# A-Kokolis/Hermes

Hardware: AMD Instinct MI355X
Metric: replicated KVS ops/s (reads+writes committed) (higher is better)
Workload: dtype u8

## Files before the change

hermes_amd/csrc/hkv_batch_dev.h:

```cpp
#pragma once
#include <hip/hip_runtime.h>

#include <type_traits>

#include "hkv_exec.h"
#include "hkv_internal.h"
#include "hkv_table_dev.h"

namespace hkv {

constexpr uint32_t kNone = 0xFFFFFFFFu;
enum : uint8_t { kStDone = 0, kStCommit = 1, kStPend = 2, kStDefer = 3 };
enum { kCtrFbM = 1, kCtrFbL = 2, kCtrDefer = 3 };

struct BatchArgs {
    uint8_t *elems;
    const int32_t *counts;
    const int32_t *offsets;
    const uint8_t *index;
    uint8_t *log;
    uint8_t *rw;
    int32_t *ns_idx;
    unsigned long long *fw;
    unsigned long long *fx, *fy;
    unsigned long long *ft;
    uint32_t fw_mask;
    uint32_t *ent;
    uint8_t *st;
    uint32_t *pf;
    uint8_t *shadow;
    unsigned long long *mem;
    uint32_t *fbl;
    uint32_t *ctr;
    unsigned int *error_flags;
    Geometry g;
    int64_t n;
    int64_t rw_stride;
    int32_t stride;
    int32_t esz;
    int32_t type;
    uint32_t rtag0;
    uint8_t ltag;
    int32_t rounds;
    int32_t inv_direct;
    int32_t ack_direct;
    uint8_t g_membership;
    uint8_t w_ack_init;
    int32_t *node_suspected;
    int32_t n_batches;
    const uint8_t *host_src;
    uint8_t *host_dst;
    uint8_t *dev_region;
    uint64_t region_bytes;
    uint32_t *done_flag;
    uint32_t done_value;
    unsigned long long *prof;
    const SmallBatch *hdr;
    uint8_t *state_out;
    const uint8_t *opc;
    const uint8_t *patch;
    uint16_t *fk;
    uint64_t *hx;
    uint8_t *rws;
    const uint8_t *rwo;
    int32_t n_rows, skip_row;
    int64_t row_stride;
    int32_t dbg;
    int32_t check_unique;
    uint8_t *ack_out;
    uint32_t ack_out_size;
    uint8_t *line;
};

enum class Engine : uint8_t {
    kSmall,
    kLocalDirect,
    kRows,
    kUniqueLds64,
    kUniqueLdsBig,
    kUniqueInPlace,
    kValsOnePass,
    kRoundsAckDirect,
    kRoundsInvDirect,
    kRoundsSlab,
    kRoundsInPlace,
};
enum class Patches : uint8_t {
    kNone,
    kApplyFirst,
    kByEngine,
    kInResolve,
};
constexpr uint32_t kPirMaxValue = 320;
constexpr uint32_t kWaveWordsMaxValue = 8 * 62;
static_assert(kPirMaxValue <= kWaveWordsMaxValue, "wave_value_copies_n ignores VCopy::fill: handle it there first");
struct BatchPlan {
    int refuse;
    Engine engine;
    Patches patches;
    int sv;
    int rmax, ch;
    int slab_threads;
    int64_t lookup_head;
    bool big;
    bool mixed;
    bool inv_direct, ack_direct;
    bool ack_out;
    bool state_out, opc;
    bool fk;
    bool rw_mirrors;
    bool node_suspected;
    bool il;
    bool inline_instance;
};

int launch_small(const BatchArgs &a, const BatchPlan &p, hipStream_t s);
int launch_local(const BatchArgs &a, const BatchPlan &p, hipStream_t s);

template <class F>
inline void with_sv(int sv, F &&f)
{
    if (sv == 31) f(std::integral_constant<int, 31>{});
    else if (sv == 287) f(std::integral_constant<int, 287>{});
    else f(std::integral_constant<int, 0>{});
}
template <class F>
inline void with_bool(bool b, F &&f)
{
    if (b) f(std::true_type{});
    else f(std::false_type{});
}

__device__ __forceinline__ Ctx make_ctx(const BatchArgs &a)
{
    Ctx c;
    c.g = a.g;
    c.g_membership = a.g_membership;
    c.w_ack_init = a.w_ack_init;
    c.rw = nullptr;
    c.rws = nullptr;
    c.rw_done = nullptr;
    c.vc = nullptr;
    return c;
}

__device__ __forceinline__ uint64_t phys_of(const BatchArgs &a, uint32_t e) { return (uint64_t)e * a.g.entry_unit; }
__device__ __forceinline__ uint8_t *entry_of(const BatchArgs &a, uint32_t e) { return a.log + phys_of(a, e); }

struct __attribute__((aligned(8))) U64x2 {
    uint64_t a, b;
};

template <int TYPE>
__device__ __forceinline__ uint8_t absorbing_state()
{
    return TYPE == kVals ? kValid : kWrite;
}

template <int TYPE>
__device__ __forceinline__ Meta after_first(const BatchArgs &a, const Meta &m0, uint32_t f, int f_is_put)
{
    Meta m1 = m0;
    m_set_state(m1, absorbing_state<TYPE>());
    if (TYPE != kLocal || a.g.skew == 0) return m1;
    uint8_t foc = f_is_put ? (uint8_t)kOpPut : a.elems[(int64_t)f * a.esz + 8];
    if (a.hx && !f_is_put) {
        const uint64_t pb = *reinterpret_cast<const uint64_t *>(a.patch + (int64_t)f * 16 + 8);
        if ((pb >> 48) & 0xFFu) foc = (uint8_t)pb;
    }
    if (foc != kOpGet) {
        m1.ver += 2;
        m_set_cid(m1, (uint8_t)a.g.machine_id);
    } else {
        m_set_state(m1, kReplay);
    }
    return m1;
}

__device__ __forceinline__ int32_t batch_of(const BatchArgs &a, int64_t i, int64_t &start)
{
    if (!a.offsets) {
        const int32_t b = (int32_t)(i / a.stride);
        start = (int64_t)b * a.stride;
        return b;
    }
    int lo = 0, hi = a.n_batches - 1;
    while (lo < hi) {
        const int mid = (lo + hi + 1) >> 1;
        if (a.offsets[mid] <= i) lo = mid; else hi = mid - 1;
    }
    start = a.offsets[lo];
    return lo;
}

constexpr int kRowsWindow = 128;
__host__ __device__ inline int32_t kary_stride(int32_t lo, int32_t hi) { return (hi - lo + 63) >> 6; }
__host__ __device__ inline int32_t kary_sample(int32_t lo, int32_t hi, int s) { return lo + (s + 1) * kary_stride(lo, hi); }
__host__ __device__ inline void kary_narrow(int32_t &lo, int32_t &hi, int32_t c)
{
    const int32_t step = kary_stride(lo, hi);
    lo += c * step;
    if (lo + step - 1 < hi) hi = lo + step - 1;
}
template <class Count>
__host__ __device__ inline int32_t kary_last_le(int32_t n, int32_t span, Count &&count)
{
    int32_t lo = 0, hi = n - 1;
    while (hi - lo > span) kary_narrow(lo, hi, count(lo, hi));
    return lo;
}

template <class Win>
__host__ __device__ inline bool rows_window_batch(Win &&win, int32_t lo, int32_t k0, int64_t i, int64_t i_max, int32_t &b)
{
    int32_t k = k0;
    for (int32_t j = k0 + 1; j < kRowsWindow; ++j) {
        const int32_t v = win(j);
        if ((int64_t)v > i_max) break;
        if ((int64_t)v <= i) k = j;
    }
    b = lo + k;
    return k + 1 < kRowsWindow;
}

__device__ __forceinline__ void batch_rw(const BatchArgs &a, int32_t b, Ctx &c)
{
    c.rw = a.rw ? a.rw + (int64_t)b * a.rw_stride : nullptr;
    c.rws = a.rws ? a.rws + (int64_t)b * (a.rw_stride / a.g.op_size) : nullptr;
    c.rwo = a.rwo ? a.rwo + (int64_t)b * (a.rw_stride / a.g.op_size) : nullptr;
}

__device__ __forceinline__ void elem_at(const BatchArgs &a, uint32_t i, uint8_t *&x, uint8_t &idx, Ctx &c)
{
    c.rw = nullptr;
    c.rws = nullptr;
    idx = 0;
    if (a.rw || !a.offsets) {
        int64_t start;
        const int32_t b = batch_of(a, i, start);
        idx = (uint8_t)(i - start);
        batch_rw(a, b, c);
    }
    x = a.elems + (int64_t)i * a.esz;
}

__device__ __forceinline__ void note_state(const BatchArgs &a, int64_t i, const uint8_t *x)
{
    if (a.state_out) a.state_out[i] = x[9];
}

__device__ __forceinline__ uint32_t fw_index(const BatchArgs &a, uint64_t phys)
{
    return (uint32_t)(((phys >> 6) * 0x9E3779B1ull) & a.fw_mask);
}
__device__ __forceinline__ unsigned long long *fw_of(const BatchArgs &a, uint32_t e) { return a.fw + fw_index(a, phys_of(a, e)); }

__device__ __forceinline__ uint32_t first_cand(unsigned long long f, uint32_t rtag)
{
    return (uint32_t)(f >> 32) == ~rtag ? (uint32_t)f : kNone;
}

__device__ __forceinline__ void offer(unsigned long long *f, uint32_t rtag, uint32_t i)
{
    const unsigned long long v = ((unsigned long long)(~rtag) << 32) | i;
    if (v < __hip_atomic_load(f, __ATOMIC_RELAXED, __HIP_MEMORY_SCOPE_AGENT)) atomicMin(f, v);
}

__device__ __forceinline__ uint8_t *shadow_of(const BatchArgs &a, uint32_t i)
{
    return a.shadow + (size_t)i * a.g.entry_size;
}

__device__ __forceinline__ void copy_entry(uint8_t *dst, const uint8_t *src, uint32_t bytes)
{
    struct __attribute__((aligned(8))) W16 {
        uint64_t a, b;
    };
    uint32_t o = 0;
    for (; o + 16 <= bytes; o += 16) *reinterpret_cast<W16 *>(dst + o) = *reinterpret_cast<const W16 *>(src + o);
    if (o < bytes) *reinterpret_cast<uint64_t *>(dst + o) = *reinterpret_cast<const uint64_t *>(src + o);
}

template <int TYPE, int SV>
__device__ __forceinline__ void apply_to_shadow(const BatchArgs &a, uint8_t *x, uint32_t i, const uint8_t *src)
{
    uint8_t *sh = shadow_of(a, i);
    Meta m;
    meta_load(src, m);
    if (SV == 31) {
        const uint4 *s4 = reinterpret_cast<const uint4 *>(src);
        uint4 *d4 = reinterpret_cast<uint4 *>(sh);
        const uint4 w0 = s4[0], w1 = s4[1], w2 = s4[2], w3 = s4[3];
        d4[0] = w0;
        d4[1] = w1;
        d4[2] = w2;
        d4[3] = w3;
    } else {
        copy_entry(sh, src, a.g.entry_size);
    }
    Ctx c = make_ctx(a);
    uint8_t *xg;
    uint8_t idx;
    elem_at(a, i, xg, idx, c);
    if (x) dispatch<SV>(TYPE, x, sh, idx, m, c);
    else dispatch<SV>(TYPE, xg, sh, idx, m, c);
    meta_store(sh, m);
}

__device__ __forceinline__ bool patch_valid(uint64_t pb) { return ((pb >> 48) & 0xFFu) != 0; }

__device__ __forceinline__ bool in_count(const BatchArgs &a, uint32_t i)
{
    if (!a.counts) return true;
    const uint32_t b = i / (uint32_t)a.stride;
    return (int32_t)(i - b * (uint32_t)a.stride) < a.counts[b];
}

__device__ __forceinline__ uint64_t line_key_meta(const uint4 &ln, Meta &m)
{
    const uint64_t ek = (uint64_t)(uint32_t)__shfl((int)ln.z, 0, 4) | ((uint64_t)(uint32_t)__shfl((int)ln.w, 0, 4) << 32);
    m.w4 = (uint32_t)__shfl((int)ln.x, 1, 4);
    m.w5 = (uint32_t)__shfl((int)ln.y, 1, 4);
    m.ver = (uint32_t)__shfl((int)ln.z, 1, 4);
    const uint32_t w7 = (uint32_t)__shfl((int)ln.w, 1, 4);
    const uint32_t b32 = (uint32_t)__shfl((int)ln.x, 2, 4) & 0xFFu;
    m.llw_cid = (uint8_t)w7;
    m.llw_ver = (w7 >> 8) | (b32 << 24);
    return ek;
}

constexpr int kLookupPair = 2;
struct NothingBeside {
    __device__ __forceinline__ void operator()() const {}
};
template <int P = kLookupPair, bool IL = false, bool F = false, class Beside = NothingBeside>
__device__ __forceinline__ void lookup_core(const BatchArgs &a, const uint64_t *key, const bool *probe, int q,
                                            int gbase, bool *ok, uint64_t *phys, uint4 *ln, unsigned long long *fwv,
                                            uint8_t **home, bool *inl, Beside &&beside = Beside{})
{
    uint4 v[P], ev[P];
#pragma unroll
    for (int k = 0; k < P; ++k) {
        if (IL) {
            const uint4 *l = line_words(a.line, bucket_of(a.g, key[k]));
            v[k] = probe[k] ? l[q] : make_uint4(0u, 0u, 0u, 0u);
            ev[k] = probe[k] ? l[4 + q] : make_uint4(0u, 0u, 0u, 0u);
        } else {
            v[k] = probe[k] ? bucket_words(a.index, bucket_of(a.g, key[k]))[q] : make_uint4(0u, 0u, 0u, 0u);
        }
    }
    beside();
    bool il[P];
#pragma unroll
    for (int k = 0; k < P; ++k) {
        const uint64_t s0 = u64_of(v[k].x, v[k].y), s1 = u64_of(v[k].z, v[k].w);
        const uint32_t tag = key_tag(key[k]);
        const bool mt0 = probe[k] && (s0 & 1u) && ((uint32_t)(s0 >> 1) & 0x7FFFFFu) == tag;
        const bool mt1 = probe[k] && (s1 & 1u) && ((uint32_t)(s1 >> 1) & 0x7FFFFFu) == tag;
        const uint32_t g0 = (uint32_t)(__ballot(mt0) >> gbase) & 0xFu;
        const uint32_t g1 = (uint32_t)(__ballot(mt1) >> gbase) & 0xFu;
        uint32_t o = 0;
#pragma unroll
        for (int l = 0; l < 4; ++l) o |= ((g0 >> l) & 1u) << (2 * l) | ((g1 >> l) & 1u) << (2 * l + 1);
        const int first = o ? __ffs(o) - 1 : 0;
        const uint64_t raw = group_slot_word(slot_off_raw(s0), slot_off_raw(s1), first), off = off_of<IL>(raw);
        ok[k] = probe[k] && o && in_log_window(a.g, off);
        phys[k] = off & a.g.log_mask;
        il[k] = off_is_inline<IL>(raw) && ok[k];
    }
#pragma unroll
    for (int k = 0; k < P; ++k) {
        if (IL) {
            ln[k] = ev[k];
            if (!il[k]) ln[k] = ok[k] ? reinterpret_cast<const uint4 *>(a.log + phys[k])[q] : make_uint4(0u, 0u, 0u, 0u);
            if (home) home[k] = il[k] ? line_entry(a.line, a.g, key[k]) : a.log + phys[k];
            if (inl) inl[k] = il[k];
        } else {
            ln[k] = ok[k] ? reinterpret_cast<const uint4 *>(a.log + phys[k])[q] : make_uint4(0u, 0u, 0u, 0u);
            if (home) home[k] = a.log + phys[k];
            if (inl) inl[k] = false;
        }
        if (F) fwv[k] = ok[k] && q == 0 ? a.fw[fw_index(a, phys[k])] : ~0ull;
    }
}

template <int P = kLookupPair, bool IL = false>
__device__ __forceinline__ void lookup_pair(const BatchArgs &a, const uint64_t *key, const bool *probe, int q,
                                            int gbase, bool *ok, uint64_t *phys, uint4 *ln, uint8_t **home = nullptr,
                                            bool *inl = nullptr)
{
    lookup_core<P, IL, false>(a, key, probe, q, gbase, ok, phys, ln, nullptr, home, inl);
}

template <int P, bool IL, class Beside>
__device__ __forceinline__ void lookup_pair_beside(const BatchArgs &a, const uint64_t *key, const bool *probe, int q,
                                                   int gbase, bool *ok, uint64_t *phys, uint4 *ln, uint8_t **home,
                                                   Beside &&beside)
{
    lookup_core<P, IL, false>(a, key, probe, q, gbase, ok, phys, ln, nullptr, home, nullptr, beside);
}

template <int P, bool IL = false>
__device__ __forceinline__ void lookup_pair_f(const BatchArgs &a, const uint64_t *key, const bool *probe, int q,
                                              int gbase, bool *ok, uint64_t *phys, uint4 *ln, unsigned long long *fwv,
                                              uint8_t **home = nullptr, bool *inl = nullptr)
{
    lookup_core<P, IL, true>(a, key, probe, q, gbase, ok, phys, ln, fwv, home, inl);
}

}
```

hermes_amd/csrc/hkv_batch_local.hip:

```cpp
#include <hip/hip_runtime.h>

#include "hkv_batch_dev.h"

namespace hkv {

#ifdef HKV_DEBUG_MODES
#define HKV_DBG_ON(a, bit) (((a).dbg & (bit)) != 0)
#else
#define HKV_DBG_ON(a, bit) false
#endif

constexpr int kPreElems = 2048;
constexpr int kPreThreads = kPreElems / 4;
constexpr int kPreHead = 1024;
constexpr int kPreHash = 2048;

constexpr uint32_t kEntInline = 0x80000000u;
template <bool IL>
__device__ __forceinline__ uint32_t ent_id(uint32_t e) { return IL ? e & ~kEntInline : e; }
template <bool IL>
__device__ __forceinline__ uint8_t *entry_home(const BatchArgs &a, uint32_t e, uint64_t key)
{
    if (IL && (e & kEntInline)) return line_entry(a.line, a.g, key);
    return entry_of(a, ent_id<IL>(e));
}

__device__ __forceinline__ uint64_t elem_key(const BatchArgs &a, int64_t i)
{
    if (a.patch && a.patch[i * 16 + 14]) return *reinterpret_cast<const uint64_t *>(a.patch + i * 16);
    return *reinterpret_cast<const uint64_t *>(a.elems + i * a.esz);
}

__device__ __forceinline__ uint4 patch_chunk(uint4 w, int q, uint64_t pa, uint64_t pb)
{
    const uint32_t fill = (uint32_t)((pb >> 32) & 0xFFu) * 0x01010101u;
    const bool vfill = fill != 0, reset = ((pb >> 40) & 0xFFu) != 0;
    if (q == 0) {
        w.x = (uint32_t)pa;
        w.y = (uint32_t)(pa >> 32);
        w.z = (uint32_t)(pb & 0xFFu) | ((uint32_t)kNew << 8) | ((uint32_t)((pb >> 8) & 0xFFu) << 16) |
              (reset ? 0u : (w.z & 0xFF000000u));
        if (reset) w.w = 0;
    } else if (q == 1) {
        const uint32_t flags = (uint32_t)((pb >> 16) & 0xFFFFu);
        w.x = flags | (vfill ? (fill & 0xFFFF0000u) : (w.x & 0xFFFF0000u));
        if (vfill) w.y = w.z = w.w = fill;
    } else if (q == 2) {
        if (vfill) w.x = w.y = w.z = w.w = fill;
    } else if (vfill) {
        w.x = (w.x & 0xFFFFFF00u) | (fill & 0xFFu);
    }
    return w;
}

__device__ __forceinline__ uint32_t pre_slot(uint64_t key)
{
    return (uint32_t)((key * 0x9E3779B97F4A7C15ull) >> (64 - __builtin_ctz(kPreHash))) & (kPreHash - 1);
}

__device__ __forceinline__ bool pre_insert(uint64_t *hk, uint32_t *hv, uint64_t key, uint32_t i, bool &created,
                                           uint32_t &slot)
{
    created = false;
    if (key == ~0ull) return false;
    uint32_t sl = pre_slot(key);
    for (int n = 0; n < kPreHash; ++n) {
        const unsigned long long old = atomicCAS((unsigned long long *)&hk[sl], ~0ull, key);
        if (old == ~0ull || old == key) {
            created = old == ~0ull;
            atomicMin(&hv[sl], i);
            slot = sl;
            return true;
        }
        sl = (sl + 1) & (kPreHash - 1);
    }
    return false;
}

__device__ __forceinline__ void pre_insert_key(uint64_t *hk, uint64_t key)
{
    if (key == ~0ull) return;
    uint32_t sl = pre_slot(key);
    for (int n = 0; n < kPreHash; ++n) {
        const unsigned long long old = atomicCAS((unsigned long long *)&hk[sl], ~0ull, key);
        if (old == ~0ull || old == key) return;
        sl = (sl + 1) & (kPreHash - 1);
    }
}

constexpr int kPrePair = 4;
template <bool IL = false>
__global__ __launch_bounds__(kPreThreads) void k_local_pre(BatchArgs a)
{
    constexpr int HEAD = kPreHead;
    __shared__ uint64_t hk[kPreHash], gk[kPreHash];
    __shared__ uint32_t hv[kPreHash];
    __shared__ uint32_t dl[kPreElems];
    __shared__ uint32_t nd;
    const int tid = threadIdx.x, q = tid & 3, gbase = (tid & 63) & ~3;
    if (tid == 0) {
        nd = 0;
        if (blockIdx.x == 0) a.ctr[kCtrDefer] = 0;
    }
    for (int j = tid; j < kPreHash; j += kPreThreads) {
        hk[j] = ~0ull;
        gk[j] = ~0ull;
        hv[j] = kNone;
    }
    if (HKV_DBG_ON(a, 8)) return;
    const int64_t i0 = (int64_t)blockIdx.x * kPreElems;
    const int64_t head_end = HKV_DBG_ON(a, 4) ? 0 : i0 < HEAD ? i0 : HEAD;
    constexpr int kOwnK = kPreElems / kPreThreads, kAllK = kOwnK + (HEAD + kPreThreads - 1) / kPreThreads;
    U64x2 h[kAllK];
    bool in[kAllK];
    uint8_t opm[kAllK];
    U64x2 pt[kAllK];
#pragma unroll
    for (int k = 0; k < kAllK; ++k) {
        const bool own = k < kOwnK;
        const int64_t i = own ? i0 + k * kPreThreads + tid : (int64_t)(k - kOwnK) * kPreThreads + tid;
        in[k] = i < a.n && (own || i < head_end);
        opm[k] = a.opc ? a.opc[in[k] ? i : 0] : (uint8_t)kOpPut;
    }
    if (a.patch) {
#pragma unroll
        for (int k = 0; k < kAllK; ++k) {
            const bool own = k < kOwnK;
            const int64_t i = own ? i0 + k * kPreThreads + tid : (int64_t)(k - kOwnK) * kPreThreads + tid;
            pt[k] = in[k] && opm[k] == kOpPut ? *reinterpret_cast<const U64x2 *>(a.patch + i * 16) : U64x2{0, 0};
        }
#pragma unroll
        for (int k = 0; k < kAllK; ++k) {
            const bool own = k < kOwnK;
            const int64_t i = own ? i0 + k * kPreThreads + tid : (int64_t)(k - kOwnK) * kPreThreads + tid;
            h[k] = *reinterpret_cast<const U64x2 *>(a.elems + (in[k] && opm[k] == kOpPut && !patch_valid(pt[k].b) ? i : 0) * 56);
        }
    } else {
#pragma unroll
        for (int k = 0; k < kAllK; ++k) {
            const bool own = k < kOwnK;
            const int64_t i = own ? i0 + k * kPreThreads + tid : (int64_t)(k - kOwnK) * kPreThreads + tid;
            h[k] = *reinterpret_cast<const U64x2 *>(a.elems + (in[k] && opm[k] == kOpPut ? i : 0) * 56);
            pt[k] = U64x2{0, 0};
        }
    }
#pragma unroll
    for (int k = 0; k < kAllK; ++k)
        if (patch_valid(pt[k].b)) {
            h[k].a = pt[k].a;
            h[k].b = (h[k].b & ~0xFFFFull) | (pt[k].b & 0xFFu) | ((uint64_t)kNew << 8);
        }
#pragma unroll
    for (int k = 0; k < kAllK; ++k) {
        const bool own = k < kOwnK;
        const int64_t i = own ? i0 + k * kPreThreads + tid : (int64_t)(k - kOwnK) * kPreThreads + tid;
        in[k] = in[k] && opm[k] == kOpPut && in_count(a, (uint32_t)i);
    }
    if (HKV_DBG_ON(a, 16)) {
        uint64_t acc = 0;
#pragma unroll
        for (int k = 0; k < kAllK; ++k) acc += h[k].a ^ h[k].b;
        if (acc == 0x1234567ull) a.ctr[7] = 1;
        return;
    }
    __syncthreads();
#pragma unroll
    for (int k = 0; k < kAllK; ++k) {
        const bool own = k < kOwnK;
        const uint32_t i = (uint32_t)(own ? i0 + k * kPreThreads + tid : (int64_t)(k - kOwnK) * kPreThreads + tid);
        const uint64_t key = h[k].a;
        if (!(in[k] && (uint8_t)h[k].b == kOpPut && !skip_elem_os(kLocal, kOpPut, (uint8_t)(h[k].b >> 8)))) continue;
        bool created;
        uint32_t sl;
        if (own) {
            const bool in_table = pre_insert(hk, hv, key, i, created, sl);
            if (!in_table || created) {
                dl[atomicAdd(&nd, 1u)] = in_table ? sl : ~i;
            }
        } else {
            pre_insert_key(gk, key);
        }
    }
    __syncthreads();
    const Ctx c = make_ctx(a);
    const uint64_t hput[2] = {0, (uint64_t)kOpPut};
    const uint32_t cnt = HKV_DBG_ON(a, 2) ? 0 : nd;
    for (uint32_t base = 0; base < cnt; base += (kPreThreads / 4) * kPrePair) {
        uint64_t key[kPrePair];
        bool probe[kPrePair], ok[kPrePair];
        uint32_t idx[kPrePair];
        uint64_t phys[kPrePair];
        uint4 ln[kPrePair];
#pragma unroll
        for (int k = 0; k < kPrePair; ++k) {
            const uint32_t j = base + k * (kPreThreads / 4) + (tid >> 2);
            probe[k] = j < cnt;
            const uint32_t d = probe[k] ? dl[j] : 0u;
            idx[k] = !probe[k] ? kNone : d < (uint32_t)kPreHash ? hv[d] : ~d;
            key[k] = !probe[k] ? 0 : d < (uint32_t)kPreHash ? hk[d] : elem_key(a, (int64_t)idx[k]);
            if (probe[k] && head_end > 0 && key[k] != ~0ull) {
                uint32_t sl = pre_slot(key[k]);
                for (int n = 0; n < kPreHash; ++n) {
                    const uint64_t g = gk[sl];
                    if (g == ~0ull) break;
                    if (g == key[k]) {
                        probe[k] = false;
                        break;
                    }
                    sl = (sl + 1) & (kPreHash - 1);
                }
            }
        }
        lookup_pair<kPrePair, IL>(a, key, probe, q, gbase, ok, phys, ln);
#pragma unroll
        for (int k = 0; k < kPrePair; ++k) {
            Meta m0;
            const uint64_t ek = line_key_meta(ln[k], m0);
            if (q != 0 || !ok[k] || ek != key[k]) continue;
            if (!would_mutate(kLocal, reinterpret_cast<const uint8_t *>(hput), m0, c) || HKV_DBG_ON(a, 1)) continue;
            atomicMin(a.fw + fw_index(a, phys[k]), ((unsigned long long)(~a.rtag0) << 32) | idx[k]);
        }
    }
}

__device__ __forceinline__ void local_resolve_nm(const BatchArgs &a, uint8_t *x, const uint8_t *ent, const Meta &m)
{
    const uint8_t oc = x[8], st = m_state(m);
    const bool obi_empty = m_obi(m) == kObiEmpty;
    bool mut = false;
    if (oc == kOpGet) {
        if (st == kValid) {
            copy_value<31>(x + kOpValueOff, ent + kEntryValueOff, 31);
            x[9] = kGetComplete;
            x[10] = (uint8_t)((m_val_len(m) >> a.g.shift) - kOpMetaSize);
        } else if (st == kInvalidWrite || st == kWrite || st == kReplay) {
            x[9] = kGetStall;
        } else {
            x[9] = kEmpty;
            if (st == kInvalid) {
                const uint8_t lw = m_lwid(m);
                if (lw < 8 && ((a.g_membership >> lw) & 1u)) x[9] = kGetStall;
                else mut = obi_empty;
            }
        }
        if (a.g.skew & kSkewReadComplete) hot_read_complete(x, m.ver, m_cid(m));
    } else if (oc == kOpPut) {
        mut = (st == kValid || st == kInvalid) && obi_empty;
        x[9] = kPutStall;
        if (a.g.skew & kSkewWriteCoalesce) {
            const uint32_t cv = m.ver & 0xFFFFu;
            uint32_t over = ld32(x + 12);
            if (st != kReplay && over == 0) {
                st32(x + 12, cv);
                over = cv;
            }
            if (over > 0 && over + 1u < cv) x[9] = kPutComplete;
        }
    }
    if (mut && a.error_flags) atomicOr(a.error_flags, 1u);
}

__device__ __forceinline__ void local_first_lds(const BatchArgs &a, uint8_t *x, uint32_t i, uint8_t *ent, Meta m)
{
    Ctx c = make_ctx(a);
    const uint8_t idx = (uint8_t)(i - i / (uint32_t)a.stride * (uint32_t)a.stride);
    if (x[8] == kOpGet) exec_read<31>(x, ent, idx, m, c);
    else if (x[8] == kOpPut) exec_write<31>(x, ent, idx, m, c);
    meta_store(ent, m);
}

constexpr int kLfWaves = 2;
template <bool IL = false>
__global__ __launch_bounds__(64 * kLfWaves) __attribute__((amdgpu_num_sgpr(80))) void k_local_fused(BatchArgs a)
{
    constexpr int P = 2, NW = kLfWaves;
    constexpr int E = 16 * P;
    constexpr int EB = E * NW;
    static_assert(EB == 64, "one wave resolves the block, one element per lane");
    __shared__ uint4 sops_b[EB * 4];
    __shared__ uint4 sln_b[EB * 4];
    __shared__ unsigned long long sfw_b[EB];
    __shared__ uint32_t sent_b[EB];
    __shared__ uint8_t sprb_b[EB];
    __shared__ uint8_t sfl[EB];
    __shared__ uint32_t sst[EB / 4], sstate[EB / 4];
    __shared__ uint32_t sdef[EB];
    __shared__ uint32_t ndef;
    const int w = threadIdx.x >> 6, tid = threadIdx.x & 63, q = tid & 3, gbase = tid & ~3;
    uint4 *sops = sops_b + w * E * 4, *sln = sln_b + w * E * 4;
    unsigned long long *sfw = sfw_b + w * E;
    uint32_t *sent = sent_b + w * E;
    uint8_t *sprb = sprb_b + w * E;
    const int64_t ib = (int64_t)blockIdx.x * EB, i0 = ib + (int64_t)w * E;
    if (threadIdx.x == 0) ndef = 0;
    uint64_t key[P];
    bool probe[P], ok[P], live[P];
    uint64_t phys[P];
    uint4 ln[P], op[P];
    int te[P];
#pragma unroll
    for (int k = 0; k < P; ++k) {
        te[k] = k * 16 + (tid >> 2);
        const int64_t i = i0 + te[k];
        live[k] = i < a.n;
        op[k] = make_uint4(0u, 0u, 0u, 0u);
        if (live[k]) {
            const uint8_t *xg = a.elems + i * 56 + 16 * q;
            U64x2 p{0, 0};
            if (a.patch) p = *reinterpret_cast<const U64x2 *>(a.patch + i * 16);
            if (q < 3) {
                op[k] = *reinterpret_cast<const uint4 *>(xg);
            } else {
                const uint64_t t = *reinterpret_cast<const uint64_t *>(xg);
                op[k].x = (uint32_t)t;
                op[k].y = (uint32_t)(t >> 32);
            }
            if (patch_valid(p.b)) op[k] = patch_chunk(op[k], q, p.a, p.b);
        }
        sops[te[k] * 4 + q] = op[k];
    }
#pragma unroll
    for (int k = 0; k < P; ++k) {
        key[k] = (uint64_t)(uint32_t)__shfl((int)op[k].x, 0, 4) | ((uint64_t)(uint32_t)__shfl((int)op[k].y, 0, 4) << 32);
        const uint32_t h0 = (uint32_t)__shfl((int)op[k].z, 0, 4);
        probe[k] = false;
        if (live[k] && !HKV_DBG_ON(a, 128))
            probe[k] = in_count(a, (uint32_t)(i0 + te[k])) && !skip_elem_os(kLocal, (uint8_t)h0, (uint8_t)(h0 >> 8));
    }
    unsigned long long fwv[P];
    bool inl[P];
    if (HKV_DBG_ON(a, 512)) {
        lookup_pair<P, IL>(a, key, probe, q, gbase, ok, phys, ln, nullptr, inl);
#pragma unroll
        for (int k = 0; k < P; ++k) fwv[k] = ~0ull;
    } else {
        lookup_pair_f<P, IL>(a, key, probe, q, gbase, ok, phys, ln, fwv, nullptr, inl);
    }
#pragma unroll
    for (int k = 0; k < P; ++k) {
        Meta m;
        const uint64_t ek = line_key_meta(ln[k], m);
        const bool hit = ok[k] && ek == key[k];
        const unsigned long long f = hit && m_state(m) != kInvalid && q == 0 ? fwv[k] : ~0ull;
        if (hit) sln[te[k] * 4 + q] = ln[k];
        if (q == 0) {
            sfw[te[k]] = f;
            sent[te[k]] = hit ? (uint32_t)(phys[k] / a.g.entry_unit) | (IL && inl[k] ? kEntInline : 0u) : kNone;
            sprb[te[k]] = probe[k];
        }
    }
    __syncthreads();
    if (__builtin_amdgcn_readfirstlane(w) == 0 && !HKV_DBG_ON(a, 64)) {
        const int64_t i = ib + tid;
        uint8_t st = kStDone;
        if (i < a.n) {
            uint8_t *x = reinterpret_cast<uint8_t *>(&sops_b[tid * 4]);
            uint8_t *ent = reinterpret_cast<uint8_t *>(&sln_b[tid * 4]);
            const uint32_t e = sent_b[tid];
            const bool prb = sprb_b[tid] != 0;
            if (e != kNone) {
                Meta m;
                meta_load(ent, m);
                Ctx c = make_ctx(a);
                const bool wm = would_mutate(kLocal, x, m, c);
                if (m_state(m) == kInvalid) {
                    if (wm) {
                        const uint64_t ph = phys_of(a, ent_id<IL>(e));
                        offer(a.fw + fw_index(a, ph), a.rtag0, (uint32_t)i);
                        if ((uint8_t)(m.w5 >> 16) != a.ltag)
                            entry_home<IL>(a, e, *reinterpret_cast<const uint64_t *>(x))[kEntryMetaOff + 4] = a.ltag;
                    }
                    st = kStDefer;
                    sdef[atomicAdd(&ndef, 1u)] = (uint32_t)i;
                } else {
                    const uint32_t f = first_cand(sfw_b[tid], a.rtag0);
                    if (wm && (f == kNone || f > (uint32_t)i) && a.error_flags) atomicOr(a.error_flags, 4u);
                    if ((uint32_t)i == f) {
                        local_first_lds(a, x, (uint32_t)i, ent, m);
                        st = kStCommit;
                    } else {
                        local_resolve_nm(a, x, ent, f != kNone && (uint32_t)i > f ? after_first<kLocal>(a, m, f, 1) : m);
                    }
                }
            } else if (prb) {
                x[9] = kMiss;
            }
            if (a.opc && prb && x[8] == kOpPut && a.opc[i] != kOpPut && a.error_flags) atomicOr(a.error_flags, 8u);
            if (!HKV_DBG_ON(a, 1024)) a.ent[i] = e;
            reinterpret_cast<uint8_t *>(sst)[tid] = st;
            reinterpret_cast<uint8_t *>(sstate)[tid] = x[9];
        }
        const unsigned long long fm = __ballot(st == kStCommit);
        if (fm && !HKV_DBG_ON(a, 1024)) {
            if (st == kStCommit) sfl[__popcll(fm & ((1ull << tid) - 1ull))] = (uint8_t)tid;
            __threadfence_block();
            const int nf = __popcll(fm);
            for (int j = tid >> 2; j < nf; j += 16) {
                const int t = sfl[j];
                reinterpret_cast<uint4 *>(shadow_of(a, (uint32_t)(ib + t)))[q] = sln_b[t * 4 + q];
            }
        }
    }
    __syncthreads();
    if (!HKV_DBG_ON(a, 1024) && !HKV_DBG_ON(a, 64)) {
        if (ib + EB <= a.n && ((uintptr_t)a.state_out & 3) == 0) {
            if ((int)threadIdx.x < EB / 4) {
                reinterpret_cast<uint32_t *>(a.st + ib)[threadIdx.x] = sst[threadIdx.x];
                if (a.state_out) reinterpret_cast<uint32_t *>(a.state_out + ib)[threadIdx.x] = sstate[threadIdx.x];
            }
        } else if ((int)threadIdx.x < EB && ib + threadIdx.x < a.n) {
            a.st[ib + threadIdx.x] = reinterpret_cast<const uint8_t *>(sst)[threadIdx.x];
            if (a.state_out) a.state_out[ib + threadIdx.x] = reinterpret_cast<const uint8_t *>(sstate)[threadIdx.x];
        }
    }
    if (ndef && threadIdx.x == 0) {
        const uint32_t base = atomicAdd(&a.ctr[kCtrDefer], ndef);
        for (uint32_t j = 0; j < ndef; ++j) a.fbl[base + j] = sdef[j];
    }
#pragma unroll
    for (int k = 0; k < P; ++k) {
        if (!live[k] || HKV_DBG_ON(a, 256)) continue;
        uint8_t *xg = a.elems + (i0 + te[k]) * 56 + 16 * q;
        const uint4 v = sops[te[k] * 4 + q];
        if (q < 3) *reinterpret_cast<uint4 *>(xg) = v;
        else *reinterpret_cast<uint64_t *>(xg) = (uint64_t)v.x | ((uint64_t)v.y << 32);
    }
}

template <bool IL = false>
__global__ __launch_bounds__(256) void k_local_deferred(BatchArgs a)
{
    const uint32_t nd = a.ctr[kCtrDefer];
    for (uint32_t j = blockIdx.x * 256u + threadIdx.x; j < nd; j += gridDim.x * 256u) {
        const uint32_t i = a.fbl[j];
        const uint32_t e = a.ent[i];
        uint8_t *xg;
        uint8_t idx;
        Ctx c = make_ctx(a);
        elem_at(a, i, xg, idx, c);
        uint8_t *entry = IL ? entry_home<IL>(a, e, *reinterpret_cast<const uint64_t *>(xg)) : entry_of(a, e);
        Meta m;
        meta_load(entry, m);
        const uint32_t f = first_cand(*fw_of(a, ent_id<IL>(e)), a.rtag0);
        uint8_t st = kStDone;
        if (f == kNone || i < f) {
            Meta tm = m;
            dispatch<31>(kLocal, xg, entry, idx, tm, c);
            if (a.error_flags && !meta_equal(tm, m)) atomicOr(a.error_flags, 1u);
        } else if (i == f) {
            apply_to_shadow<kLocal, 31>(a, nullptr, i, entry);
            st = kStCommit;
        } else {
            const Meta m1 = after_first<kLocal>(a, m, f, 0);
            Meta tm = m1;
            dispatch<31>(kLocal, xg, entry, idx, tm, c);
            if (a.error_flags && !meta_equal(tm, m1)) atomicOr(a.error_flags, 1u);
        }
        a.st[i] = st;
        note_state(a, i, xg);
    }
}

constexpr int kCwElems = 1024;
template <bool IL = false>
__global__ __launch_bounds__(256) void k_commit_w(BatchArgs a)
{
    __shared__ uint32_t lst[4][kCwElems];
    const int lane = threadIdx.x & 63, w = threadIdx.x >> 6;
    const int64_t e0 = ((int64_t)blockIdx.x * 4 + w) * kCwElems + 16 * lane;
    uint32_t m = 0;
    if (e0 + 16 <= a.n) {
        const uint4 s4 = *reinterpret_cast<const uint4 *>(a.st + e0);
        const uint32_t sw[4] = {s4.x, s4.y, s4.z, s4.w};
#pragma unroll
        for (int b = 0; b < 16; ++b)
            if (((sw[b >> 2] >> (8 * (b & 3))) & 0xFFu) == kStCommit) m |= 1u << b;
    } else {
        for (int b = 0; b < 16; ++b)
            if (e0 + b < a.n && a.st[e0 + b] == kStCommit) m |= 1u << b;
    }
    const uint32_t c = __popc(m);
    uint32_t incl = c;
#pragma unroll
    for (int d = 1; d < 64; d <<= 1) {
        const uint32_t v = (uint32_t)__shfl_up((int)incl, d, 64);
        if (lane >= d) incl += v;
    }
    const uint32_t total = (uint32_t)__shfl((int)incl, 63, 64);
    for (uint32_t pos = incl - c; m; m &= m - 1) lst[w][pos++] = (uint32_t)e0 + (uint32_t)(__ffs(m) - 1);
    __syncthreads();
    const int q = lane & 3;
    for (uint32_t j = (uint32_t)(lane >> 2); j < total; j += 16) {
        const uint32_t i = lst[w][j];
        const uint4 v = reinterpret_cast<const uint4 *>(shadow_of(a, i))[q];
        if (IL) {
            const uint64_t key = (uint64_t)(uint32_t)__shfl((int)v.z, 0, 4) | ((uint64_t)(uint32_t)__shfl((int)v.w, 0, 4) << 32);
            reinterpret_cast<uint4 *>(entry_home<IL>(a, a.ent[i], key))[q] = v;
        } else {
            reinterpret_cast<uint4 *>(entry_of(a, a.ent[i]))[q] = v;
        }
    }
}

template <bool IL>
static void launch_local_il(const BatchArgs &a, hipStream_t s)
{
    const int64_t n = a.n;
    const dim3 pgrid((unsigned)((n + kPreElems - 1) / kPreElems));
    const dim3 fgrid((unsigned)((n + 32 * kLfWaves - 1) / (32 * kLfWaves)));
    hipLaunchKernelGGL(k_local_pre<IL>, pgrid, dim3(kPreThreads), 0, s, a);
    hipLaunchKernelGGL(k_local_fused<IL>, fgrid, dim3(64 * kLfWaves), 0, s, a);
    hipLaunchKernelGGL(k_local_deferred<IL>, dim3(128u), dim3(256), 0, s, a);
    hipLaunchKernelGGL(k_commit_w<IL>, dim3((unsigned)((n + 4 * kCwElems - 1) / (4 * kCwElems))), dim3(256), 0, s, a);
}

int launch_local(const BatchArgs &a, const BatchPlan &p, hipStream_t s)
{
    if (p.il) launch_local_il<true>(a, s);
    else launch_local_il<false>(a, s);
    return hipGetLastError() == hipSuccess ? 0 : -3;
}

}
```

Measured before the change: 5.226 billion.

## Compact committed shadow records per block and drop per-element state writes

The fused local kernel now packs each block's first-writer shadow images at the front of the block's record area. It writes only a per-block count instead of per-element status bytes and per-element entry ids. Deferred elements are emitted as packed records (index, entry, back slot) into a.mem, and late commits go to a separate list counted by a new counter. The commit kernel scans per-block counts with a prefix sum and binary search rather than scanning every element's status byte. This cuts global write traffic and commit-scan cost, at the price of more complex indexing and reusing the mem/fbl/pf buffers.

```diff
diff --git a/hermes_amd/csrc/hkv_batch_dev.h b/hermes_amd/csrc/hkv_batch_dev.h
--- a/hermes_amd/csrc/hkv_batch_dev.h
+++ b/hermes_amd/csrc/hkv_batch_dev.h
@@ -11,7 +11,7 @@
 
 constexpr uint32_t kNone = 0xFFFFFFFFu;
 enum : uint8_t { kStDone = 0, kStCommit = 1, kStPend = 2, kStDefer = 3 };
-enum { kCtrFbM = 1, kCtrFbL = 2, kCtrDefer = 3 };
+enum { kCtrFbM = 1, kCtrFbL = 2, kCtrDefer = 3, kCtrLate = 4 };
 
 struct BatchArgs {
     uint8_t *elems;
@@ -271,6 +271,26 @@
     return a.shadow + (size_t)i * a.g.entry_size;
 }
 
+constexpr int kRecBlock = 64;
+__host__ __device__ inline int64_t rec_blocks(int64_t n) { return (n + kRecBlock - 1) / kRecBlock; }
+__host__ __device__ inline int rec_live(int64_t n, int64_t ib) { return n - ib < kRecBlock ? (int)(n - ib) : kRecBlock; }
+__host__ __device__ inline uint32_t rec_front_slot(int64_t ib, int rank) { return (uint32_t)(ib + rank); }
+__host__ __device__ inline uint32_t rec_back_slot(int64_t ib, int live, int r) { return (uint32_t)(ib + live - 1 - r); }
+template <class Incl>
+__host__ __device__ inline int rec_find(Incl &&incl, uint32_t k, int &rank)
+{
+    int lo = 0, hi = kRecBlock - 1;
+#pragma unroll
+    for (int s = 0; s < 6; ++s) {
+        const int mid = (lo + hi) >> 1;
+        if (incl(mid) > k) hi = mid;
+        else lo = mid + 1;
+    }
+    const uint32_t before = incl(lo ? lo - 1 : 0);
+    rank = (int)(k - (lo ? before : 0u));
+    return lo;
+}
+
 __device__ __forceinline__ void copy_entry(uint8_t *dst, const uint8_t *src, uint32_t bytes)
 {
     struct __attribute__((aligned(8))) W16 {
@@ -282,9 +302,8 @@
 }
 
 template <int TYPE, int SV>
-__device__ __forceinline__ void apply_to_shadow(const BatchArgs &a, uint8_t *x, uint32_t i, const uint8_t *src)
-{
-    uint8_t *sh = shadow_of(a, i);
+__device__ __forceinline__ void apply_to_shadow_at(const BatchArgs &a, uint8_t *x, uint32_t i, const uint8_t *src, uint8_t *sh)
+{
     Meta m;
     meta_load(src, m);
     if (SV == 31) {
@@ -305,6 +324,11 @@
     if (x) dispatch<SV>(TYPE, x, sh, idx, m, c);
     else dispatch<SV>(TYPE, xg, sh, idx, m, c);
     meta_store(sh, m);
+}
+template <int TYPE, int SV>
+__device__ __forceinline__ void apply_to_shadow(const BatchArgs &a, uint8_t *x, uint32_t i, const uint8_t *src)
+{
+    apply_to_shadow_at<TYPE, SV>(a, x, i, src, shadow_of(a, i));
 }
 
 __device__ __forceinline__ bool patch_valid(uint64_t pb) { return ((pb >> 48) & 0xFFu) != 0; }
diff --git a/hermes_amd/csrc/hkv_batch_local.hip b/hermes_amd/csrc/hkv_batch_local.hip
--- a/hermes_amd/csrc/hkv_batch_local.hip
+++ b/hermes_amd/csrc/hkv_batch_local.hip
@@ -100,7 +100,10 @@
     const int tid = threadIdx.x, q = tid & 3, gbase = (tid & 63) & ~3;
     if (tid == 0) {
         nd = 0;
-        if (blockIdx.x == 0) a.ctr[kCtrDefer] = 0;
+        if (blockIdx.x == 0) {
+            a.ctr[kCtrDefer] = 0;
+            a.ctr[kCtrLate] = 0;
+        }
     }
     for (int j = tid; j < kPreHash; j += kPreThreads) {
         hk[j] = ~0ull;
@@ -276,23 +279,26 @@
     constexpr int P = 2, NW = kLfWaves;
     constexpr int E = 16 * P;
     constexpr int EB = E * NW;
-    static_assert(EB == 64, "one wave resolves the block, one element per lane");
+    static_assert(EB == 64 && EB == kRecBlock, "one wave resolves the block, one element per lane; a block is a record area");
     __shared__ uint4 sops_b[EB * 4];
     __shared__ uint4 sln_b[EB * 4];
     __shared__ unsigned long long sfw_b[EB];
     __shared__ uint32_t sent_b[EB];
     __shared__ uint8_t sprb_b[EB];
     __shared__ uint8_t sfl[EB];
-    __shared__ uint32_t sst[EB / 4], sstate[EB / 4];
+    __shared__ uint32_t sstate[EB / 4];
     __shared__ uint32_t sdef[EB];
-    __shared__ uint32_t ndef;
+    __shared__ uint32_t ndef, nfs;
     const int w = threadIdx.x >> 6, tid = threadIdx.x & 63, q = tid & 3, gbase = tid & ~3;
     uint4 *sops = sops_b + w * E * 4, *sln = sln_b + w * E * 4;
     unsigned long long *sfw = sfw_b + w * E;
     uint32_t *sent = sent_b + w * E;
     uint8_t *sprb = sprb_b + w * E;
     const int64_t ib = (int64_t)blockIdx.x * EB, i0 = ib + (int64_t)w * E;
-    if (threadIdx.x == 0) ndef = 0;
+    if (threadIdx.x == 0) {
+        ndef = 0;
+        nfs = 0;
+    }
     uint64_t key[P];
     bool probe[P], ok[P], live[P];
     uint64_t phys[P];
@@ -352,7 +358,7 @@
     __syncthreads();
     if (__builtin_amdgcn_readfirstlane(w) == 0 && !HKV_DBG_ON(a, 64)) {
         const int64_t i = ib + tid;
-        uint8_t st = kStDone;
+        bool first = false;
         if (i < a.n) {
             uint8_t *x = reinterpret_cast<uint8_t *>(&sops_b[tid * 4]);
             uint8_t *ent = reinterpret_cast<uint8_t *>(&sln_b[tid * 4]);
@@ -370,14 +376,13 @@
                         if ((uint8_t)(m.w5 >> 16) != a.ltag)
                             entry_home<IL>(a, e, *reinterpret_cast<const uint64_t *>(x))[kEntryMetaOff + 4] = a.ltag;
                     }
-                    st = kStDefer;
-                    sdef[atomicAdd(&ndef, 1u)] = (uint32_t)i;
+                    sdef[atomicAdd(&ndef, 1u)] = (uint32_t)tid;
                 } else {
                     const uint32_t f = first_cand(sfw_b[tid], a.rtag0);
                     if (wm && (f == kNone || f > (uint32_t)i) && a.error_flags) atomicOr(a.error_flags, 4u);
                     if ((uint32_t)i == f) {
                         local_first_lds(a, x, (uint32_t)i, ent, m);
-                        st = kStCommit;
+                        first = true;
                     } else {
                         local_resolve_nm(a, x, ent, f != kNone && (uint32_t)i > f ? after_first<kLocal>(a, m, f, 1) : m);
                     }
@@ -386,36 +391,39 @@
                 x[9] = kMiss;
             }
             if (a.opc && prb && x[8] == kOpPut && a.opc[i] != kOpPut && a.error_flags) atomicOr(a.error_flags, 8u);
-            if (!HKV_DBG_ON(a, 1024)) a.ent[i] = e;
-            reinterpret_cast<uint8_t *>(sst)[tid] = st;
             reinterpret_cast<uint8_t *>(sstate)[tid] = x[9];
         }
-        const unsigned long long fm = __ballot(st == kStCommit);
-        if (fm && !HKV_DBG_ON(a, 1024)) {
-            if (st == kStCommit) sfl[__popcll(fm & ((1ull << tid) - 1ull))] = (uint8_t)tid;
-            __threadfence_block();
-            const int nf = __popcll(fm);
-            for (int j = tid >> 2; j < nf; j += 16) {
-                const int t = sfl[j];
-                reinterpret_cast<uint4 *>(shadow_of(a, (uint32_t)(ib + t)))[q] = sln_b[t * 4 + q];
-            }
-        }
+        const unsigned long long fm = __ballot(first);
+        if (first) sfl[__popcll(fm & ((1ull << tid) - 1ull))] = (uint8_t)tid;
+        if (tid == 0) nfs = (uint32_t)__popcll(fm);
     }
     __syncthreads();
-    if (!HKV_DBG_ON(a, 1024) && !HKV_DBG_ON(a, 64)) {
+    const bool rec = !HKV_DBG_ON(a, 1024) && !HKV_DBG_ON(a, 64);
+    const int nf = rec ? (int)nfs : 0;
+    for (int j = (int)threadIdx.x >> 2; j < nf; j += 16 * NW)
+        reinterpret_cast<uint4 *>(shadow_of(a, rec_front_slot(ib, j)))[q] = sln_b[sfl[j] * 4 + q];
+    if ((int)threadIdx.x < nf) a.ent[rec_front_slot(ib, (int)threadIdx.x)] = sent_b[sfl[threadIdx.x]];
+    if (threadIdx.x == 64) a.st[blockIdx.x] = (uint8_t)nf;
+    if (rec && a.state_out) {
         if (ib + EB <= a.n && ((uintptr_t)a.state_out & 3) == 0) {
-            if ((int)threadIdx.x < EB / 4) {
-                reinterpret_cast<uint32_t *>(a.st + ib)[threadIdx.x] = sst[threadIdx.x];
-                if (a.state_out) reinterpret_cast<uint32_t *>(a.state_out + ib)[threadIdx.x] = sstate[threadIdx.x];
-            }
+            if ((int)threadIdx.x < EB / 4) reinterpret_cast<uint32_t *>(a.state_out + ib)[threadIdx.x] = sstate[threadIdx.x];
         } else if ((int)threadIdx.x < EB && ib + threadIdx.x < a.n) {
-            a.st[ib + threadIdx.x] = reinterpret_cast<const uint8_t *>(sst)[threadIdx.x];
-            if (a.state_out) a.state_out[ib + threadIdx.x] = reinterpret_cast<const uint8_t *>(sstate)[threadIdx.x];
-        }
-    }
-    if (ndef && threadIdx.x == 0) {
-        const uint32_t base = atomicAdd(&a.ctr[kCtrDefer], ndef);
-        for (uint32_t j = 0; j < ndef; ++j) a.fbl[base + j] = sdef[j];
+            a.state_out[ib + threadIdx.x] = reinterpret_cast<const uint8_t *>(sstate)[threadIdx.x];
+        }
+    }
+    if (ndef && w == 0) {
+        uint32_t base = 0;
+        if (tid == 0) base = atomicAdd(&a.ctr[kCtrDefer], ndef);
+        base = (uint32_t)__shfl((int)base, 0, 64);
+        if ((uint32_t)tid < ndef) {
+            const uint32_t t = sdef[tid];
+            uint4 r;
+            r.x = (uint32_t)(ib + t);
+            r.y = sent_b[t];
+            r.z = rec_back_slot(ib, rec_live(a.n, ib), tid);
+            r.w = 0;
+            reinterpret_cast<uint4 *>(a.mem)[base + tid] = r;
+        }
     }
 #pragma unroll
     for (int k = 0; k < P; ++k) {
@@ -432,8 +440,8 @@
 {
     const uint32_t nd = a.ctr[kCtrDefer];
     for (uint32_t j = blockIdx.x * 256u + threadIdx.x; j < nd; j += gridDim.x * 256u) {
-        const uint32_t i = a.fbl[j];
-        const uint32_t e = a.ent[i];
+        const uint64_t r0 = a.mem[2 * (size_t)j], r1 = a.mem[2 * (size_t)j + 1];
+        const uint32_t i = (uint32_t)r0, e = (uint32_t)(r0 >> 32), slot = (uint32_t)r1;
         uint8_t *xg;
         uint8_t idx;
         Ctx c = make_ctx(a);
@@ -442,44 +450,43 @@
         Meta m;
         meta_load(entry, m);
         const uint32_t f = first_cand(*fw_of(a, ent_id<IL>(e)), a.rtag0);
-        uint8_t st = kStDone;
         if (f == kNone || i < f) {
             Meta tm = m;
             dispatch<31>(kLocal, xg, entry, idx, tm, c);
             if (a.error_flags && !meta_equal(tm, m)) atomicOr(a.error_flags, 1u);
         } else if (i == f) {
-            apply_to_shadow<kLocal, 31>(a, nullptr, i, entry);
-            st = kStCommit;
+            apply_to_shadow_at<kLocal, 31>(a, nullptr, i, entry, shadow_of(a, slot));
+            const uint32_t l = atomicAdd(&a.ctr[kCtrLate], 1u);
+            a.fbl[l] = slot;
+            a.pf[l] = e;
         } else {
             const Meta m1 = after_first<kLocal>(a, m, f, 0);
             Meta tm = m1;
             dispatch<31>(kLocal, xg, entry, idx, tm, c);
             if (a.error_flags && !meta_equal(tm, m1)) atomicOr(a.error_flags, 1u);
         }
-        a.st[i] = st;
         note_state(a, i, xg);
     }
 }
 
-constexpr int kCwElems = 1024;
+constexpr int kCwThreads = 256;
+template <bool IL>
+__device__ __forceinline__ void commit_image(const BatchArgs &a, uint32_t slot, uint32_t e, int q)
+{
+    const uint4 v = reinterpret_cast<const uint4 *>(shadow_of(a, slot))[q];
+    if (IL) {
+        const uint64_t key = (uint64_t)(uint32_t)__shfl((int)v.z, 0, 4) | ((uint64_t)(uint32_t)__shfl((int)v.w, 0, 4) << 32);
+        reinterpret_cast<uint4 *>(entry_home<IL>(a, e, key))[q] = v;
+    } else {
+        reinterpret_cast<uint4 *>(entry_of(a, e))[q] = v;
+    }
+}
 template <bool IL = false>
-__global__ __launch_bounds__(256) void k_commit_w(BatchArgs a)
-{
-    __shared__ uint32_t lst[4][kCwElems];
-    const int lane = threadIdx.x & 63, w = threadIdx.x >> 6;
-    const int64_t e0 = ((int64_t)blockIdx.x * 4 + w) * kCwElems + 16 * lane;
-    uint32_t m = 0;
-    if (e0 + 16 <= a.n) {
-        const uint4 s4 = *reinterpret_cast<const uint4 *>(a.st + e0);
-        const uint32_t sw[4] = {s4.x, s4.y, s4.z, s4.w};
-#pragma unroll
-        for (int b = 0; b < 16; ++b)
-            if (((sw[b >> 2] >> (8 * (b & 3))) & 0xFFu) == kStCommit) m |= 1u << b;
-    } else {
-        for (int b = 0; b < 16; ++b)
-            if (e0 + b < a.n && a.st[e0 + b] == kStCommit) m |= 1u << b;
-    }
-    const uint32_t c = __popc(m);
+__global__ __launch_bounds__(kCwThreads) void k_commit_w(BatchArgs a)
+{
+    const int lane = threadIdx.x & 63, q = lane & 3, g = threadIdx.x >> 2;
+    const int64_t b0 = (int64_t)blockIdx.x * kRecBlock, nb = rec_blocks(a.n);
+    const uint32_t c = b0 + lane < nb ? a.st[b0 + lane] : 0u;
     uint32_t incl = c;
 #pragma unroll
     for (int d = 1; d < 64; d <<= 1) {
@@ -487,19 +494,19 @@
         if (lane >= d) incl += v;
     }
     const uint32_t total = (uint32_t)__shfl((int)incl, 63, 64);
-    for (uint32_t pos = incl - c; m; m &= m - 1) lst[w][pos++] = (uint32_t)e0 + (uint32_t)(__ffs(m) - 1);
-    __syncthreads();
-    const int q = lane & 3;
-    for (uint32_t j = (uint32_t)(lane >> 2); j < total; j += 16) {
-        const uint32_t i = lst[w][j];
-        const uint4 v = reinterpret_cast<const uint4 *>(shadow_of(a, i))[q];
-        if (IL) {
-            const uint64_t key = (uint64_t)(uint32_t)__shfl((int)v.z, 0, 4) | ((uint64_t)(uint32_t)__shfl((int)v.w, 0, 4) << 32);
-            reinterpret_cast<uint4 *>(entry_home<IL>(a, a.ent[i], key))[q] = v;
-        } else {
-            reinterpret_cast<uint4 *>(entry_of(a, a.ent[i]))[q] = v;
-        }
-    }
+    const auto incl_of = [&](int b) { return (uint32_t)__shfl((int)incl, b, 64); };
+    for (uint32_t k0 = 0; k0 < total; k0 += kCwThreads / 4) {
+        const uint32_t k = k0 + (uint32_t)g;
+        int rank;
+        const int b = rec_find(incl_of, k, rank);
+        if (k < total) {
+            const uint32_t slot = rec_front_slot((b0 + b) * kRecBlock, rank);
+            commit_image<IL>(a, slot, a.ent[slot], q);
+        }
+    }
+    const uint32_t nl = a.ctr[kCtrLate];
+    for (uint32_t j = blockIdx.x * (kCwThreads / 4) + (uint32_t)g; j < nl; j += gridDim.x * (kCwThreads / 4))
+        commit_image<IL>(a, a.fbl[j], a.pf[j], q);
 }
 
 template <bool IL>
@@ -511,7 +518,8 @@
     hipLaunchKernelGGL(k_local_pre<IL>, pgrid, dim3(kPreThreads), 0, s, a);
     hipLaunchKernelGGL(k_local_fused<IL>, fgrid, dim3(64 * kLfWaves), 0, s, a);
     hipLaunchKernelGGL(k_local_deferred<IL>, dim3(128u), dim3(256), 0, s, a);
-    hipLaunchKernelGGL(k_commit_w<IL>, dim3((unsigned)((n + 4 * kCwElems - 1) / (4 * kCwElems))), dim3(256), 0, s, a);
+    const int64_t cgroups = (rec_blocks(n) + kRecBlock - 1) / kRecBlock;
+    hipLaunchKernelGGL(k_commit_w<IL>, dim3((unsigned)cgroups), dim3(kCwThreads), 0, s, a);
 }
 
 int launch_local(const BatchArgs &a, const BatchPlan &p, hipStream_t s)
```

Measured after the change: 5.258 billion (median of 6 runs). Within noise of the previous version (+0.6%).
